# willow-ahrens/ChainPartitioners.jl

Measured on AMD Instinct MI355X. Metric: partitions/sec, DynamicTotalSplitter(AffineConnectivityModel{Int64}(0,0,0,1)), K=64, higher is better.
Workload: dtype int64; 1 GPU; config 3: DynamicTotalSplitter(AffineConnectivityModel{Int64}(0,0,0,1)) on suitesparse_shaped CSR (seeded SplitMix64 generator, tests/synth.py), n=10000000 rows, nnz=100000000, K=64; one independent partition per GPU; n=10000000, nnz=100000000, K=64, includes_oracle_build=True, device_block_pool=True

## Files before the change

chainpartitioners.jl_amd/csrc/capi.hip:

```cpp
#include "csr.hpp"
#include "model.hpp"
#include "dp.hpp"
#include "weight.hpp"
#include "sym.hpp"
#include <cmath>
#include <memory>

using namespace cpk;

namespace cpk {

__global__ void __launch_bounds__(256) k_range_counts(int64_t nq, const int64_t *__restrict__ P, const int64_t *__restrict__ Rr,
                                                      const int64_t *__restrict__ pos, const int32_t *__restrict__ prev,
                                                      const int64_t *__restrict__ fpos, const int32_t *__restrict__ flast,
                                                      unsigned long long *__restrict__ nets, unsigned long long *__restrict__ selfnets)
{
    int64_t i = blockIdx.x;
    if (i >= nq) return;
    __shared__ int64_t sh[256];
    int64_t p = P[i], r = Rr[i];
    int64_t stride = (int64_t)gridDim.y * 256, start = (int64_t)blockIdx.y * 256 + threadIdx.x;
    int64_t c = 0;
    if (r > p) {
        int64_t q0 = pos[p], q1 = pos[r];
// ... 54 lines not shown
        hp[i] = j[i] - 1; hr[i] = jp[i] - 1;
    }
    DBuf<int64_t> dP((size_t)nq), dR((size_t)nq), dK, dN, dS;
    DBuf<TC> dO((size_t)nq);
    CP_HIP(hipMemcpyAsync(dP.p, hp.data(), sizeof(int64_t) * (size_t)nq, hipMemcpyHostToDevice, s));
    CP_HIP(hipMemcpyAsync(dR.p, hr.data(), sizeof(int64_t) * (size_t)nq, hipMemcpyHostToDevice, s));
    if (k) { dK.alloc((size_t)nq); CP_HIP(hipMemcpyAsync(dK.p, k, sizeof(int64_t) * (size_t)nq, hipMemcpyHostToDevice, s)); }
    if (has_nets) {
        dN.alloc((size_t)nq);
        CP_HIP(hipMemsetAsync(dN.p, 0, dN.bytes(), s));
        if (need_self) { dS.alloc((size_t)nq); CP_HIP(hipMemsetAsync(dS.p, 0, dS.bytes(), s)); }
        int64_t per = nq > 0 ? A->N / nq : 0;
        unsigned gy = (unsigned)(per / 65536 + 1);
        if (gy > 2048) gy = 2048;
        ProfScope ps(PROF_QUERY, s, 0.0);
        hipLaunchKernelGGL(k_range_counts, dim3((unsigned)nq, gy), dim3(256), 0, s, nq, dP.p, dR.p, A->pos.p, A->prev.p,
                           need_self ? A->fpos.p : nullptr, need_self ? A->flast.p : nullptr, (unsigned long long *)dN.p,
                           need_self ? (unsigned long long *)dS.p : nullptr);
    }
    HostModel<TC> HM;
    build_dev_model<TC>(mdl, HM, s);
    hipLaunchKernelGGL(HIP_KERNEL_NAME(k_apply_model<TC>), dim3((unsigned)cdiv(nq, 256)), dim3(256), 0, s, nq, dP.p, dR.p,
                       k ? dK.p : nullptr, A->pos.p, has_nets ? dN.p : nullptr, need_self ? dS.p : nullptr, HM.d, dO.p);
    CP_HIP(hipGetLastError());
    CP_HIP(hipMemcpyAsync(out, dO.p, sizeof(TC) * (size_t)nq, hipMemcpyDeviceToHost, s));
    CP_HIP(hipStreamSynchronize(s));
    prof_collect();
    return CP_OK;
}

static int64_t fld(int64_t a, int64_t b)
{
    int64_t q = a / b, r = a % b;
    if (r != 0 && ((r < 0) != (b < 0))) q -= 1;
    return q;
}
static double fld(double a, int64_t b) { return std::floor(a / (double)b); }
static int64_t max_identity(int64_t) { return INT64_MIN; }
static double max_identity(double) { return -INFINITY; }
static void also_f64(const int64_t *lo, const int64_t *hi, double *lo_f64, double *hi_f64) { *lo_f64 = (double)*lo; *hi_f64 = (double)*hi; }
static void also_f64(const double *, const double *, double *, double *) {}

template <typename TC>
static int32_t oracle_eval_into(cp_csr_t A, const cp_model_t *model, const cp_rowpart_t *Pi, int64_t nq, const int64_t *j, const int64_t *jp,
                                const int64_t *k, TC *out)
{
    const bool i64 = std::is_same<TC, int64_t>::value;
    return cp_oracle_eval(A, model, Pi, CP_HINT_STEP, nq, j, jp, k, i64 ? (int64_t *)out : nullptr, i64 ? nullptr : (double *)out);
}

static const struct { const char *name; int64_t *var; bool kept; } g_stats[] = {
    {"spec_redo", &g_spec_redo, false}, {"poison_hits", &g_poison_hits, false}, {"fix_trips", &g_fix_trips, false},
    {"fix_edges", &g_fix_edges, false}, {"fix_items", &g_fix_items, false}, {"bn_sym_layers", &g_bn_sym_layers, true},
    {"own_split_tiles", &g_own_split_tiles, false},
};
static void stats_reset(bool all) { for (const auto &c : g_stats) if (all || !c.kept) *c.var = 0; }

enum OptRule { OPT_PLAIN, OPT_BOOL, OPT_CLAMP, OPT_POW2 };
constexpr int64_t NOLIM_LO = INT64_MIN, NOLIM_HI = INT64_MAX;
static const struct Opt { const char *name; int64_t *var; OptRule rule; int64_t lo, hi; } g_options[] = {
    {"force_brute", &g_opt_force_brute, OPT_PLAIN, 0, 0}, {"brute_max_n", &g_opt_brute_max_n, OPT_PLAIN, 0, 0}, {"dbg", &g_opt_dbg, OPT_PLAIN, 0, 0},
    {"short_t", &g_opt_short_t, OPT_PLAIN, 0, 0}, {"short_e", &g_opt_short_e, OPT_PLAIN, 0, 0}, {"ra_cache", &g_opt_ra_cache, OPT_PLAIN, 0, 0},
    {"leaf", &g_opt_leaf, OPT_PLAIN, 0, 0}, {"block_tables", &g_opt_block_tables, OPT_PLAIN, 0, 0}, {"nospec", &g_opt_nospec, OPT_PLAIN, 0, 0},
    {"rpass_small_tau", &g_opt_rpass_small_tau, OPT_PLAIN, 0, 0}, {"fixed_point", &g_opt_fixed_point, OPT_PLAIN, 0, 0},
    {"bn_wave", &g_opt_bn_wave, OPT_PLAIN, 0, 0},
    {"poison", &g_opt_poison, OPT_PLAIN, 0, 0},
    {"pool", &g_opt_pool, OPT_BOOL, 0, 0},
    {"own_blk", &g_opt_own_blk, OPT_BOOL, 0, 0},
    {"own_split", &g_opt_own_split, OPT_BOOL, 0, 0},
    {"lws", &g_opt_lws, OPT_BOOL, 0, 0},
    {"gap_tau", &g_opt_gap_tau, OPT_CLAMP, NOLIM_LO, 20}, {"gap_min", &g_opt_gap_min, OPT_CLAMP, 8, NOLIM_HI}, {"gap_nr", &g_opt_gap_nr, OPT_CLAMP, 1, 2},
    {"force_max", &g_opt_force_max, OPT_CLAMP, 0, NOLIM_HI}, {"rpass_cap", &g_opt_rpass_cap, OPT_CLAMP, 1, NOLIM_HI},
    {"own_min", &g_opt_own_min, OPT_CLAMP, 64, NOLIM_HI}, {"bn_chunk", &g_opt_bn_chunk, OPT_CLAMP, 1, NOLIM_HI},
    {"bn_slack", &g_opt_bn_slack, OPT_CLAMP, 0, NOLIM_HI}, {"bn_run", &g_opt_bn_run, OPT_CLAMP, 2, NOLIM_HI},
    {"rpass_ch", &g_opt_rpass_ch, OPT_POW2, 16, 4096}, {"setup_bs", &g_opt_setup_bs, OPT_POW2, 64, 1024}, {"lws_leaf", &g_opt_lws_leaf, OPT_POW2, 256, 2048},
};
static int64_t opt_value(const Opt &o, int64_t value)
{
    switch (o.rule) {
    case OPT_BOOL: return value ? 1 : 0;
    case OPT_CLAMP: return value < o.lo ? o.lo : value > o.hi ? o.hi : value;
    case OPT_POW2: { int64_t v = o.lo; while (v < value && v < o.hi) v <<= 1; return v; }
    default: return value;
    }
}

}

extern "C" {

const char *cp_last_error(void) { return g_last_error.c_str(); }
int32_t cp_version(void) { return 100; }

int32_t cp_device_count(void)
{
    int c = 0;
    if (hipGetDeviceCount(&c) != hipSuccess) return 0;
    return c;
}

static int32_t csr_create_impl(int64_t m, int64_t n, int64_t N, const int64_t *colptr, const int64_t *rowval,
                               int32_t device, bool on_device, cp_csr_t *out)
{
    return guarded([&]() -> int32_t {
        CP_REQUIRE(out && colptr && (rowval || N == 0), CP_EINVAL, "null argument");
        CP_REQUIRE(m >= 0 && n >= 0 && N >= 0, CP_EINVAL, "negative dimension");
        CP_REQUIRE(n < (int64_t)1 << 30 && m < (int64_t)1 << 30 && N < ((int64_t)1 << 31) - 65536, CP_EINVAL,
                   "dimensions exceed the 32-bit link-array layout");
        CP_REQUIRE(cp_device_count() > 0, CP_EHIP, "no HIP device visible: libchainpart has no CPU fallback");
        CP_HIP(hipSetDevice(device));
        std::unique_ptr<cp_csr_s> A(new cp_csr_s());
        A->device = device; A->m = m; A->n = n; A->N = N;
        CP_HIP(hipStreamCreate(&A->stream));
        A->own_stream = true;
        csr_upload(A.get(), colptr, rowval, on_device);
        *out = A.release();
        return CP_OK;
    });
}

int32_t cp_csr_create(int64_t m, int64_t n, int64_t N, const int64_t *colptr, const int64_t *rowval, int32_t device, cp_csr_t *out)
{
// ... 510 lines not shown
```

chainpartitioners.jl_amd/csrc/dp.hpp:

```cpp
#pragma once
#include "csr.hpp"
#include "model.hpp"

struct cp_dp_s {
    cp_csr_s *A = nullptr;
    int64_t K = 0;
    int32_t combine = 0, order = 0;
    bool fast = false, fast_bn = false, need_self = false;
    void *work = nullptr;
    cpk::DBuf<int32_t> ptr;
    int64_t rlo = 0, rhi = 0;
    int64_t wwin = 0;
    std::vector<int64_t> lay_lo, lay_hi;
    virtual ~cp_dp_s() = default;
    virtual int32_t step_layer(int64_t k, const void *cst_prev_device, void *cst_cur_device) = 0;
    virtual int32_t block_tables(int32_t *nplanes_out, int64_t *opt_out, int64_t *nets_out, int64_t *selfnets_out) = 0;
};

namespace cpk {

using DpBase = ::cp_dp_s;

struct DpWindow {
    int64_t w = 0;
// ... 37 lines not shown
                         int64_t wwin = 0, int64_t p_lo0 = 0, int64_t p_hi0 = -1, const int32_t *j0 = nullptr,
                         const BnPattern *pat = nullptr);
extern int64_t g_opt_bn_wave, g_opt_bn_run, g_opt_bn_slack;
extern int64_t g_opt_bn_chunk;

template <typename TC>
int32_t run_dyn_constrained(cp_csr_s *A, int64_t K, int32_t g, int32_t order, const cp_model_t *mdl, const cp_rowpart_t *Pi,
                            const cp_model_t *w, int64_t wi, double wf, int64_t *spl_out);
template <typename TC>
int32_t run_seq_eval(cp_csr_s *A, const cp_model_t *mdl, const cp_rowpart_t *Pi, int64_t nq, const int64_t *j, const int64_t *jp,
                     const int64_t *k, TC *out);

template <typename TC>
int32_t run_plaid_eval(cp_csr_s *A, const cp_model_t *mdl, const cp_rowpart_t *Pi, int64_t nq, const int64_t *j, const int64_t *jp,
                       const int64_t *k, TC *out);
template <typename TC>
int32_t run_plaid_dynamic(cp_csr_s *A, int64_t K, int32_t combine, int32_t order, const cp_model_t *mdl, const cp_rowpart_t *Pi,
                          int64_t *spl_out);

template <typename TC>
bool pack_dynamic_scan(hipStream_t s, int64_t n, int64_t wmax, const TC *Ftab, TC *cst1, int64_t *spl1);

extern int64_t g_opt_lws, g_opt_lws_leaf;
bool lws_ok(const cp_csr_s *A, const cp_model_t *mdl, const cp_model_t *w, int64_t wi, double wf);
template <typename TC>
int32_t run_pack_lws(cp_csr_s *A, const DevModel<TC> &M, const WaveletDev &wnet, const WaveletDev &wself, const cp_model_t *w, int64_t wi,
                     double wf, TC *cst1, int64_t *spl1);

extern int64_t g_opt_gap_nr;
extern int64_t g_opt_gap_tau, g_opt_gap_min;
extern int64_t g_opt_poison, g_poison_hits;
void dp_round_scans_test(const int32_t *a, int64_t na, int64_t na_max, const int32_t *b, int64_t nb, int64_t nb_max, int two, int64_t capT, int64_t capNT,
                         int err_in, int reps, int64_t *offs_out, int64_t *toffs_out, int64_t *res);
void dp_fix_merge_test(const cp_model_t *model, int64_t ntask, const int64_t *toffs, const int64_t *part_v, const int32_t *part_p, const int32_t *part_nn,
                       const int32_t *part_nl, const int32_t *tile_s, const int32_t *tile_s2, const int32_t *anchor, const int32_t *anchor2, const int32_t *row,
                       const int32_t *plane, int64_t n, int reps, int32_t *p_out, int32_t *nn_out, int32_t *nl_out, int64_t *res);
extern int64_t g_fix_trips, g_fix_edges;
extern int64_t g_fix_items;
extern int64_t g_opt_leaf;
extern int64_t g_opt_block_tables;
extern int64_t g_opt_ra_cache;
extern int64_t g_opt_fixed_point;
extern int64_t g_opt_nospec;
extern int64_t g_spec_redo;
extern int64_t g_opt_rpass_small_tau;
extern int64_t g_opt_force_max;
extern int64_t g_opt_setup_bs;
extern int64_t g_opt_rpass_cap;
extern int64_t g_opt_rpass_ch;
extern int64_t g_opt_own_min;
extern int64_t g_opt_own_blk;
extern int64_t g_opt_own_split;
extern int64_t g_own_split_tiles;
void dp_own_split_test(cp_csr_s *A, int32_t *vpos_out, int32_t *vsa_out, int32_t *vnext_out, int64_t *res);
extern int64_t g_opt_short_t, g_opt_short_e;
extern int64_t g_opt_force_brute;
extern int64_t g_opt_brute_max_n;
extern int64_t g_opt_dbg;
enum DbgBit : int64_t {
    DBG_PRINT_ROUNDS = 8,
    DBG_NO_INTERIOR = 32,
    DBG_NO_OWN_TILES = 64,
    DBG_POISON = 128,
    DBG_POISON_ZERO = 256,
    DBG_GAP_ALL_SPECIAL = 512,
    DBG_MISPREDICT = 1024,
    DBG_TINY_BUFFERS = 2048,
    DBG_COUNT_NONTRIVIAL = 4096,
    DBG_COMBINE_BY_SLOT = 16384,
    DBG_RA_ROWMAJOR = 262144,
    DBG_NO_FORCE_OWN = 524288,
    DBG_WIN_NO_RA_CACHE = 1048576,
    DBG_WIN_NO_MIR_CACHE = 2097152,
    DBG_BN_NO_HINT2 = 4194304,
    DBG_MIR_ROWMAJOR = 8388608,
    DBG_RA_ALL_LEVELS = 33554432,
    DBG_BN_NO_HINT_STARTS = 33554432,
};

}
```

chainpartitioners.jl_amd/csrc/dp_brute.hip:

```cpp
#include "csr.hpp"
#include "model.hpp"
#include "dp.hpp"

namespace cpk {

int64_t g_opt_force_brute = 0;
int64_t g_opt_short_t = 8, g_opt_short_e = 64;
int64_t g_opt_own_min = 64;
int64_t g_opt_own_blk = 1;
int64_t g_opt_own_split = 1;
int64_t g_own_split_tiles = 0;
int64_t g_opt_rpass_ch = 256;
int64_t g_opt_rpass_small_tau = 4;
int64_t g_opt_force_max = 1024;
int64_t g_opt_setup_bs = 1024;
int64_t g_opt_rpass_cap = 200;
int64_t g_opt_nospec = 0, g_spec_redo = 0;
int64_t g_opt_gap_tau = 6, g_opt_gap_min = 64, g_opt_gap_nr = 2;
int64_t g_opt_ra_cache = 1;
int64_t g_opt_leaf = 1, g_opt_block_tables = 0;
int64_t g_opt_poison = 0, g_poison_hits = 0;
int64_t g_fix_trips = 0, g_fix_edges = 0, g_fix_items = 0;
int64_t g_opt_fixed_point = 0;
int64_t g_opt_brute_max_n = 200000;
int64_t g_opt_dbg = 0;

template <typename TC>
__global__ void __launch_bounds__(256) k_brute_layer(int64_t n, int64_t r_lo, int64_t r_hi, const int64_t *__restrict__ pos,
                                                     const int32_t *__restrict__ next, const int64_t *__restrict__ fpos,
                                                     const int32_t *__restrict__ flast, DevModel<TC> M, TC alpha,
                                                     int32_t g, const TC *__restrict__ W, TC *__restrict__ cst,
                                                     int32_t *__restrict__ ptr)
{
    int64_t wave = ((int64_t)blockIdx.x * blockDim.x + threadIdx.x) >> 6;
    int lane = threadIdx.x & 63;
    int64_t r0 = r_lo + wave * 64;
    if (r0 > r_hi) return;
    int64_t r = r0 + lane;
    bool live = r <= r_hi;
    int64_t rtop = r0 + 63 < r_hi ? r0 + 63 : r_hi;
    int64_t nn = 0, nl = 0;
    TC best = (TC)0;
    int64_t bp = -1;
    bool self = (M.kind == CP_MODEL_HYPEREDGE_CUT);
    int32_t rr = (int32_t)r;
    for (int64_t p = rtop; p >= 0; p--) {
        if (p < n) {
            bool step = live && (r > p);
            int64_t q0 = pos[p], q1 = pos[p + 1];
            for (int64_t q = q0; q < q1; q++) {
                int32_t nx = next[q];
                if (step) nn += (nx >= rr);
            }
            if (self) {
                int64_t s0 = fpos[p], s1 = fpos[p + 1];
                for (int64_t sidx = s0; sidx < s1; sidx++) {
                    int32_t la = flast[sidx];
                    if (step) nl += (la < rr);
                }
            }
        }
        if (live && r >= p) {
            TC f = dm_apply(M, alpha, r - p, pos[r] - pos[p], nn, nl);
            TC v = comb(g, W[p], f);
// ... 25 lines not shown
```

chainpartitioners.jl_amd/csrc/dp_total.hip:

```cpp
#include "csr.hpp"
#include "model.hpp"
#include "dp.hpp"
#include <algorithm>

namespace cpk {

template <typename TC>
__device__ __forceinline__ TC dm_apply_affine(const DevModel<TC> &m, TC alpha, int64_t nv, int64_t np, int64_t nn, int64_t nl)
{
    TC v = cadd(cadd(alpha, cmulc(nv, m.p[CP_P_VERTEX])), cmulc(np, m.p[CP_P_PIN]));
    if (m.kind == CP_MODEL_CONNECTIVITY) return cadd(v, cmulc(nn, m.p[CP_P_NET]));
    if (m.kind == CP_MODEL_HYPEREDGE_CUT) return cadd(cadd(v, cmulc(nl, m.p[CP_P_SELF_NET])), cmulc(nn - nl, m.p[CP_P_CUT_NET]));
    return v;
}
#define dm_apply dm_apply_affine

constexpr int LT = 256;
constexpr int NBMAX = 31;
constexpr int SPLIT_BMIN = 8;
constexpr int SPLIT_NB = NBMAX - SPLIT_BMIN;

__device__ __forceinline__ int64_t prow(int64_t r, int64_t n)
{
    int t = __ffsll((long long)r) - 1;
// ... 771 lines not shown
        if (hi > re) hi = re;
        if (hi > n + 1) hi = n + 1;
        gap_hi[tile] = (int32_t)hi;
    }
    }
}

__global__ void __launch_bounds__(256) k_blk_order(const RoundCounts *__restrict__ rc, const int4 *__restrict__ rec, const int32_t *__restrict__ brank,
                                                   const int64_t *__restrict__ bstart, int32_t *__restrict__ border, int4 *__restrict__ srec,
                                                   int32_t *__restrict__ bcnt)
{
    const int64_t ntile = rc->NT;
    for (int64_t tile = (int64_t)blockIdx.x * blockDim.x + threadIdx.x; tile < ntile; tile += (int64_t)gridDim.x * blockDim.x) {
        const int4 r = rec[tile];
        const int32_t c = r.x / LT, rk = brank[tile];
        const int64_t slot = bstart[c] + rk;
        border[slot] = (int32_t)tile;
        srec[slot] = r;
        if (rk == 0) bcnt[c] = 0;
    }
}

template <typename TC, bool HYP, bool GAP>
__global__ void __launch_bounds__(256) k_lpass_own(int isA, const RoundCounts *__restrict__ rc, const int32_t *__restrict__ border,
                                                   const int32_t *__restrict__ a_pos, const int32_t *__restrict__ a_next,
                                                   const int32_t *__restrict__ a_fpos, const int32_t *__restrict__ a_flast,
                                                   int32_t *__restrict__ a_tileS, int32_t *__restrict__ a_tileS2, const int4 *__restrict__ a_rec,
                                                   const int4 *__restrict__ a_srec, const TC *__restrict__ W, DevModel<TC> M, TC alpha, Best<TC, HYP> *__restrict__ part,
                                                   int tau, const int32_t *__restrict__ gap_hi, uint8_t *__restrict__ spec, int force_spec,
                                                   Best<TC, HYP> *__restrict__ sub, int32_t *__restrict__ spv,
                                                   const int32_t *__restrict__ a_col, const int32_t *__restrict__ a_ffirst,
                                                   const int32_t *__restrict__ a_vnext, const int32_t *__restrict__ a_vpos,
                                                   const int32_t *__restrict__ a_vsa, int64_t vstride)
{
    int lane = threadIdx.x & 63;
    int64_t tile = (int64_t)blockIdx.x * 4 + __builtin_amdgcn_readfirstlane(threadIdx.x >> 6);
    if (tile >= rc->NT) return;
    const int4 vrec = border ? a_srec[tile] : a_rec[tile];
    if (border) tile = border[tile];
    const int32_t rw = __builtin_amdgcn_readfirstlane(vrec.w);
    const int4 rec = make_int4(__builtin_amdgcn_readfirstlane(vrec.x), __builtin_amdgcn_readfirstlane(vrec.y), __builtin_amdgcn_readfirstlane(vrec.z), rw);
    int head = rw & 1;
    int32_t tl = (rw >> 2) & 255;
    int32_t acc[4], acc2[4] = {0, 0, 0, 0}, sk[4], sk2[4];
    __shared__ int32_t s_es_all[4][2][SMAX + 1], s_v_all[4][2][SMAX + 1];
    __shared__ int32_t s_cnt_all[4];
    int32_t(*s_es)[SMAX + 1] = s_es_all[threadIdx.x >> 6], (*s_v)[SMAX + 1] = s_v_all[threadIdx.x >> 6];
    int ns = 0;
    if (GAP && (rw & 2)) {
        int32_t *s_cnt = &s_cnt_all[threadIdx.x >> 6];
        if (lane == 0) *s_cnt = 0;
        __threadfence_block();
        int32_t rL = rec.y - (1 << tau), hi1 = gap_hi[tile] - 1;
        interior_stream<true, true>(a_next, a_pos, rec.x, tl, hi1, lane, acc, sk, head, rL, hi1, s_es[0], s_v[0], s_cnt, 0);
        if (HYP) interior_stream<false, true>(a_flast, a_fpos, rec.x, tl, rL + 1, lane, acc2, sk2, head, rL, hi1, s_es[0], s_v[0], s_cnt, 1);
        __threadfence_block();
        ns = *s_cnt;
        if (force_spec) ns = SMAX + 1;
        if (ns > 0 && ns <= SMAX) {
            if (lane < ns) {
                const int32_t q = s_es[0][lane];
                const bool k1 = s_v[0][lane] < 0;
                s_es[0][lane] = rec.x - (k1 ? a_ffirst[q] : a_col[q]);
            }
            __threadfence_block();
        }
    } else if (!HYP && !GAP) {
        const int sb = rw >> 10;
        const int64_t so = sb ? (int64_t)(sb - SPLIT_BMIN) * vstride : 0;
        interior_stream<true>(sb ? a_vnext : a_next, sb ? a_vpos + so : a_pos, rec.x, tl, rec.y, lane, acc, sk, head, 0, 0, nullptr, nullptr, nullptr, 0,
                              sb ? a_vsa + so : (const int32_t *)nullptr);
#pragma unroll
        for (int k = 0; k < 4; k++) { const int32_t e = lane + 64 * k; sk[k] = (a_pos + (rec.x - tl))[(uint32_t)(tl - (e < tl ? e : tl)) & 255u]; }
    } else {
        interior_stream<true>(a_next, a_pos, rec.x, tl, rec.y, lane, acc, sk, head);
        if (HYP) interior_stream<false>(a_flast, a_fpos, rec.x, tl, rec.y, lane, acc2, sk2, head);
    }
    TC wv[4];
#pragma unroll
    for (int k = 0; k < 4; k++) { const int32_t e = lane + 64 * k; wv[k] = (W + (rec.x - tl))[(uint32_t)(tl - (e < tl ? e : tl)) & 255u]; }
    int sel = tl >> 6;
    if (lane == (tl & 63)) {
        a_tileS[tile] = sel == 0 ? acc[0] : sel == 1 ? acc[1] : sel == 2 ? acc[2] : acc[3];
        if (HYP) a_tileS2[tile] = sel == 0 ? acc2[0] : sel == 1 ? acc2[1] : sel == 2 ? acc2[2] : acc2[3];
    }
    Best<TC, HYP> cand[4];
#pragma unroll
    for (int k = 0; k < 4; k++) {
        int32_t e = lane + 64 * k;
        best_clear(cand[k]);
        if (e <= tl && !(head && isA && e == 0)) {
            int32_t p = rec.x - e;
            TC fv = dm_apply(M, alpha, (int64_t)(rec.y - p), (int64_t)(rec.z - sk[k]), (int64_t)acc[k], (int64_t)acc2[k]);
            cand[k].v = cadd(wv[k], fv); cand[k].p = p; cand[k].nn = acc[k]; best_set_nl(cand[k], acc2[k]);
        }
    }
    if (GAP && ns > SMAX) {
        if (lane == 0) spec[tile] = 255;
        return;
    }
    if (!GAP || ns == 0) {
        Best<TC, HYP> best; best_clear(best);
#pragma unroll
        for (int k = 0; k < 4; k++) best = better(best, cand[k]);
        for (int o = 32; o > 0; o >>= 1) {
            int src = (lane + o) & 63;
            Best<TC, HYP> c; best_clear(c); c.v = shfl64(best.v, src); c.p = __shfl(best.p, src); c.nn = __shfl(best.nn, src);
            if (HYP) best_set_nl(c, __shfl(best_nl(best), src));
            bool take = (best.p < 0) ? (c.p >= 0) : (c.p >= 0 && (c.v < best.v || (c.v == best.v && c.p > best.p)));
            if (lane + o < 64 && take) best = c;
        }
        if (lane == 0) { part[tile] = best; if (GAP) spec[tile] = 0; }
        return;
    }
    __threadfence_block();
    if (lane < ns) {
        int32_t es_i = s_es[0][lane]; int rank = 0;
        for (int j = 0; j < ns; j++) { int32_t es_j = s_es[0][j]; rank += (es_j < es_i) || (es_j == es_i && j < lane); }
// ... 2038 lines not shown
            dim3 sgrid((unsigned)cdiv(R.ntask, sbs));
            if (!R.isA) {
                int64_t mx = 1;
                for (int bb = R.tau + 1; bb < nbits; bb++) mx = std::max<int64_t>(mx, R.tbase[bb + 1] - R.tbase[bb]);
                sgrid = dim3((unsigned)cdiv(mx, sbs), (unsigned)std::max(1, nbits - R.tau - 1));
            }
            hipLaunchKernelGGL(HIP_KERNEL_NAME(k_setup_short<TC, HYP>), sgrid, dim3(sbs), 0, s, R, Wk.opt.p, Wk.nnopt.p, Wk.nlopt.p, Wk.cr.p, Wk.crl.p, A->pos32.p,
                               A->next.p, if_hyp<HYP>(A->fpos32.p), if_hyp<HYP>(A->flast.p), W, M, alpha, Wk.tdesc.p, Wk.tb.p, Wk.len.p, Wk.tS0l.p, &rc->nlong,
                               (int32_t)g_opt_short_t, (int32_t)g_opt_short_e, own_tiles ? Wk.o_tdesc.p : (int4 *)nullptr, Wk.o_tb.p, Wk.o_rlen.p, Wk.o_ntl.p,
                               Wk.o_tS0l.p, &rc->nown, &rc->own_steps, (int32_t)(forced ? 2 : gap ? g_opt_gap_min : g_opt_own_min),
                               (int32_t)std::min<size_t>(Wk.o_ntl.n, (size_t)INT32_MAX), &rc->err, Wk.fin.p, Wk.last_s0.p,
                               (g_opt_dbg & DBG_COUNT_NONTRIVIAL) ? &rc->_pad : (int32_t *)nullptr, Wk.w_anch.p, Wk.w_anch2.p, pzp, oblk);
        }
        RoundCounts P;
        if (spec) {
            P = Wk.pred[(size_t)rd];
            if (Wk.pred_scale != 1.0) {
                auto sc = [&](int64_t v) { return (int64_t)((double)v * Wk.pred_scale) + (v > 0 ? 1 : 0); };
                P.nlong = (int32_t)sc(P.nlong); P.nown = (int32_t)sc(P.nown); P.T = sc(P.T); P.NT = sc(P.NT);
                P.own_steps = (unsigned long long)sc((int64_t)P.own_steps);
            }
            if ((g_opt_dbg & DBG_MISPREDICT) && (rd & 1)) { P.nown = 0; P.NT = 0; P.nlong = 0; P.T = 0; }
            Wk.ensure_own((size_t)grow(P.NT));
            Wk.ensure_flat((size_t)grow(P.T));
        }
        {
            ProfScope ps(PROF_SCAN, s, 12.0 * (double)R.ntask);
            const bool tiny = spec && (g_opt_dbg & DBG_TINY_BUFFERS);
            const int64_t capT = spec ? (tiny ? (int64_t)64 : (int64_t)Wk.loc.n) : INT64_MAX, capNT = spec ? (tiny ? (int64_t)1 : (int64_t)Wk.o_rec.n) : INT64_MAX;
            const int64_t nm = std::min<int64_t>(R.ntask, (int64_t)Wk.o_ntl.n);
            if (R.ntask <= LB_MAX) {
                launch_round_scans(rc, Wk.len.p, Wk.offs.p, R.ntask, Wk.o_ntl.p, Wk.o_toffs.p, nm, own_tiles, capT, capNT, Wk.scanws, s);
            } else {
                exclusive_scan_i32_devn(Wk.len.p, Wk.offs.p, &rc->nlong, R.ntask, &rc->T, Wk.scratch, s);
                if (own_tiles) exclusive_scan_i32_devn(Wk.o_ntl.p, Wk.o_toffs.p, &rc->nown, nm, &rc->NT, Wk.scratch, s);
                hipLaunchKernelGGL(k_round_finish, dim3(1), dim3(1), 0, s, rc, capT, capNT);
            }
        }
        if (!spec) {
            CP_HIP(hipMemcpyAsync(&P, rc, sizeof(P), hipMemcpyDeviceToHost, s));
            CP_HIP(hipStreamSynchronize(s));
            Wk.ensure_own((size_t)P.NT);
            Wk.ensure_flat((size_t)P.T);
        }
        used[(size_t)rd] = P;
        if (g_opt_dbg & DBG_PRINT_ROUNDS) fprintf(stderr, "round isA=%d tau=%d ntask=%lld %s long=%d own=%d T=%lld NT=%lld nontrivial=%d\n", R.isA, R.tau, (long long)R.ntask,
                                   spec ? "predicted" : "exact", P.nlong, P.nown, (long long)P.T, (long long)P.NT, P._pad);
        if (P.nown > 0 && P.NT > 0) {
            const int64_t gNT = spec ? (int64_t)Wk.o_rec.n : P.NT, gown = spec ? grow(P.nown) : P.nown;
            poison_fill(s, {{Wk.o_part.p, Wk.o_part.bytes()}, {Wk.o_tileS.p, Wk.o_tileS.bytes()}, {Wk.o_rec.p, Wk.o_rec.bytes()}, {Wk.o_srec.p, Wk.o_srec.bytes()},
                            {if_hyp<HYP>(Wk.o_tileS2.p), Wk.o_tileS2.bytes()}, {Wk.o_items.p, Wk.o_items.bytes()}, {Wk.o_item_of.p, Wk.o_item_of.bytes()},
                            {Wk.o_trec.p, Wk.o_trec.bytes()}});
            const unsigned mgrid = (unsigned)std::min<int64_t>(cdiv(gNT, 256), 8192);
            const int split = !(split_layer && !gap && !R.isA) ? 0 : R.tau + 1 >= SPLIT_BMIN ? 1 : 2;
            split_mode[(size_t)rd] = (int8_t)split;
            if (split && !Wk.split.built) {
                ProfScope ps(PROF_LINKS, s, 8.0 * (double)A->N + 16.0 * (double)(nbits - SPLIT_BMIN) * (double)(n + 1));
                split_build(A, Wk.split, Wk.scratch);
            }
            hipLaunchKernelGGL(k_own_map, dim3(mgrid), dim3(256), 0, s, rc, Wk.o_toffs.p, Wk.o_tdesc.p, Wk.o_rlen.p, Wk.o_rec.p, Wk.o_task.p,
                               Wk.o_tb.p, gap ? Wk.o_hi.p : (int32_t *)nullptr, R.tau, n, oblk, oblk ? Wk.b_cnt.p : (int32_t *)nullptr, Wk.o_brank.p,
                               gap ? (int2 *)nullptr : Wk.o_items.p, Wk.o_item_of.p, split);
            {
                ProfScope ps(gap ? PROF_GAPSTREAM : PROF_OWN, s, own_bytes(R.tau, split != 0, (double)P.own_steps));
                if (oblk) {
                    exclusive_scan_i32_lb(Wk.b_cnt.p, Wk.b_start.p, Wk.b_n.p, Wk.b_nblk, nullptr, Wk.scanws, s);
                    hipLaunchKernelGGL(k_blk_order, dim3(mgrid), dim3(256), 0, s, rc, Wk.o_rec.p, Wk.o_brank.p, Wk.b_start.p, Wk.o_border.p, Wk.o_srec.p, Wk.b_cnt.p);
                }
                hipLaunchKernelGGL(HIP_KERNEL_NAME(gap ? k_lpass_own<TC, HYP, true> : k_lpass_own<TC, HYP, false>), dim3((unsigned)cdiv(gNT, 4)), dim3(256), 0, s,
                                   R.isA, rc,
                                   oblk ? Wk.o_border.p : (const int32_t *)nullptr, A->pos32.p, A->next.p, if_hyp<HYP>(A->fpos32.p), if_hyp<HYP>(A->flast.p),
                                   Wk.o_tileS.p, Wk.o_tileS2.p, Wk.o_rec.p, Wk.o_srec.p, W, M, alpha, recs<HYP>(Wk.o_part), R.tau, Wk.o_hi.p, Wk.o_spec.p,
                                   (int)((g_opt_dbg & DBG_GAP_ALL_SPECIAL) != 0), recs<HYP>(Wk.o_sub), Wk.o_spv.p, A->col.p, if_hyp<HYP>(A->ffirst.p),
                                   split ? Wk.split.vnext.p : (const int32_t *)nullptr, Wk.split.vpos.p, Wk.split.vsa.p, (int64_t)(n + 1));
            }
            note(rd, 0, gap ? PROF_GAPSTREAM : PROF_OWN, R.tau, split != 0);
            if (gap) {
                {
                    ProfScope ps(PROF_CARRY, s, 12.0 * (double)P.NT);
                    const int32_t *ntp = reinterpret_cast<const int32_t *>(&rc->NT);
                    exclusive_scan_i32_lb(Wk.o_tileS.p, Wk.o_tilePS.p, ntp, (int64_t)Wk.o_tileS.n, nullptr, Wk.scanws, s);
                    if (hyp) exclusive_scan_i32_lb(Wk.o_tileS2.p, Wk.o_tilePS2.p, ntp, (int64_t)Wk.o_tileS.n, nullptr, Wk.scanws, s);
                }
                ProfScope ps(PROF_GAP, s, 24.0 * (double)P.NT);
                const int nchunk = (int)std::max<int64_t>(1, ((int64_t)2 << R.tau) / 64);
                const size_t ncap = Wk.o_rec.n / GAPSEG + 2;
                Wk.g_list.ensure(ncap); Wk.g_slot.ensure(2 * ncap);
                Wk.g_seg.ensure((2 * ncap) * (size_t)nchunk * 64 * sizeof(GapSegRec<TC, true>));
                Wk.g_slow.ensure((size_t)gown * (size_t)nchunk + 64); Wk.g_sslow.ensure((2 * ncap) * (size_t)nchunk + 64);
                CP_REQUIRE((int64_t)gown * nchunk < INT32_MAX && (int64_t)(2 * ncap) * nchunk < INT32_MAX, CP_EINTERNAL, "gap work index beyond 32 bits");
                const int gnr = (g_opt_gap_nr >= 2 && nchunk >= 2) ? 2 : 1;
                unsigned gg = (unsigned)std::min<int64_t>(cdiv(gown * cdiv((int64_t)nchunk, gnr), 4), 16384);
                unsigned gs_grid = (unsigned)std::min<int64_t>(cdiv((int64_t)(2 * ncap) * nchunk, 4), 8192);
                unsigned gm = (unsigned)std::min<int64_t>(cdiv((int64_t)ncap * nchunk, 4), 4096);
                const unsigned gslow_grid = 2048;
                launch_gap<TC, HYP>(s, A, Wk, R.tau, nchunk, gnr, rc, n, W, M, alpha, gg, gs_grid, gm, gslow_grid, oblk);
            } else {
                ProfScope ps(PROF_FIX, s, 24.0 * (double)P.NT);
                launch_fix_own<TC, HYP>(s, rc, Wk.o_toffs.p, recs<HYP>(Wk.o_part), Wk.o_tdesc.p, Wk.o_tb.p, if_hyp<HYP>(Wk.o_tS0l.p), Wk.o_tileS.p,
                                        if_hyp<HYP>(Wk.o_tileS2.p), M, Wk.opt.p, Wk.nnopt.p, if_hyp<HYP>(Wk.nlopt.p), n, Wk.o_items.p, Wk.o_item_of.p, Wk.o_trec.p,
                                        Wk.o_tick.p, spec ? grow(P.NT) : P.NT, gown);
            }
            CP_HIP(hipGetLastError());
        }
        if (P.nlong <= 0 || P.T <= 0) continue;
        const int64_t gtile = spec ? (int64_t)Wk.tileS.n : cdiv(P.T, LT);
        poison_fill(s, {{Wk.loc.p, Wk.loc.bytes()}, {if_hyp<HYP>(Wk.loc2.p), Wk.loc2.bytes()}, {Wk.partL.p, Wk.partL.bytes()}, {Wk.partR.p, Wk.partR.bytes()},
                        {Wk.tileS.p, Wk.tileS.bytes()}, {if_hyp<HYP>(Wk.tileS2.p), Wk.tileS2.bytes()}});
// ... 37 lines not shown
            CP_REQUIRE(need <= 25, CP_EINTERNAL, "leaf pass: more outer planes than counters");
            const int32_t lcap = (gaps && g_opt_gap_tau >= LEAF_T) ? (int32_t)std::max<int64_t>(g_opt_gap_min, 2) : INT32_MAX;
            LeafArgs<TC, HYP> L{};
            L.n = n; L.g0 = g0; L.ngroups = g1 - g0 + 1; L.c0 = c0; L.c1 = c1; L.nbits = nbits; L.planes = (int32_t)(g_opt_block_tables != 0);
            L.pos = A->pos32.p; L.prev = A->prev.p; L.next = A->next.p; L.col = A->col.p;
            L.fpos = if_hyp<HYP>(A->fpos32.p); L.flast = if_hyp<HYP>(A->flast.p); L.ffirst = if_hyp<HYP>(A->ffirst.p);
            L.lpos = if_hyp<HYP>(A->lpos32.p); L.lfirst = if_hyp<HYP>(A->lfirst.p);
            L.opt = Wk.opt.p; L.nnopt = Wk.nnopt.p; L.nlopt = if_hyp<HYP>(Wk.nlopt.p); L.fin = Wk.fin.p; L.fin_stamp = Wk.fin_stamp;
            L.W = W; L.M = M; L.alpha = alpha; L.cst = cst_out; L.ptr = ptr_out; L.G = G;
            L.anchM = Wk.leaf_anch.p; L.anchM2 = if_hyp<HYP>(Wk.leaf_anch2.p); L.lcap = lcap; L.err = &Wk.rc.p->err; L.pz = pzp;
            constexpr int WPB = LeafWPB<HYP>::v;
            hipLaunchKernelGGL(HIP_KERNEL_NAME(need <= 18 ? k_leaf<TC, HYP, 18> : k_leaf<TC, HYP, 25>), dim3((unsigned)cdiv(L.ngroups, WPB)), dim3(64 * WPB), 0, s, L);
            CP_HIP(hipGetLastError());
        }
    }
    {
        ProfScope ps(PROF_COMBINE, s, 24.0 * (double)(leaf ? (n >> LEAF_T) + 1 : n + 1));
        const int64_t c0 = rlo > 0 ? rlo : 0, c1 = rhi < n ? rhi : n;
        const int64_t r0 = leaf ? (c0 + LEAF_G - 1) >> LEAF_T : c0, r1 = leaf ? c1 >> LEAF_T : c1;
        const int lvl = (!leaf && (g_opt_dbg & DBG_COMBINE_BY_SLOT)) ? (2 * (c1 - c0 + 1) >= n + 1) : 0;
        const int sh = leaf ? LEAF_T : 0;
        const int32_t *nl = if_hyp<HYP>(Wk.nlopt.p);
        if (c1 >= c0 && r1 >= r0) {
            const unsigned cgrid = (unsigned)cdiv(lvl ? n + 1 : r1 - r0 + 1, 256);
            if (G.win) hipLaunchKernelGGL(HIP_KERNEL_NAME(k_combine_win<TC>), dim3(cgrid), dim3(256), 0, s, lvl, G, n, r0, r1, A->pos32.p, Wk.opt.p, Wk.nnopt.p, nl, W, M,
                                          alpha, cst_out, ptr_out, sh, pzp);
            else hipLaunchKernelGGL(HIP_KERNEL_NAME(k_combine<TC>), dim3(cgrid), dim3(256), 0, s, lvl, n, r0, r1, nbits, A->pos32.p, Wk.opt.p, Wk.nnopt.p, nl, W, M, alpha,
                                    cst_out, ptr_out, sh, pzp);
        }
    }
    CP_HIP(hipGetLastError());
    std::vector<RoundCounts> got((size_t)NR);
    int32_t pz_hits[2] = {0, 0};
    CP_HIP(hipMemcpyAsync(got.data(), Wk.rc.p, sizeof(RoundCounts) * (size_t)NR, hipMemcpyDeviceToHost, s));
    if (pzp) CP_HIP(hipMemcpyAsync(pz_hits, pzp, sizeof(pz_hits), hipMemcpyDeviceToHost, s));
    CP_HIP(hipStreamSynchronize(s));
    bool ok = true;
    for (int rd = 0; rd < NR; rd++) {
        const RoundCounts &g = got[(size_t)rd], &u = used[(size_t)rd];
        CP_REQUIRE(!(g.err && !spec && !any_forced), CP_EINTERNAL, "DP work list overflow");
        if (g.err) ok = false;
        if (g.nown > 0 && g.NT > 0 && !(u.nown > 0 && u.NT > 0)) ok = false;
        if (g.nlong > 0 && g.T > 0 && !(u.nlong > 0 && u.T > 0)) ok = false;
    }
    if (pzp) {
        g_poison_hits += pz_hits[0];
        CP_REQUIRE(!(ok && pz_hits[0] > 0), CP_EINTERNAL, "a DP layer that is not redone read plane cells nobody wrote (poison mode)");
    }
    if (ok) Wk.b_dirty = false;
    Wk.t_dirty = false;
    if (ok) for (int rd = 0; rd < NR; rd++) { g_fix_trips += got[(size_t)rd].n_trips; g_fix_edges |= got[(size_t)rd].n_edge; }
    if (ok) for (int rd = 0; rd < NR; rd++) {
        const RoundCounts &g = got[(size_t)rd];
        if (g.nown > 0 && g.NT > 0) g_own_split_tiles += split_mode[(size_t)rd] == 1 ? g.NT : split_mode[(size_t)rd] == 2 ? g.n_split : 0;
    }
    for (int rd = 0; rd < NR; rd++) g_fix_items += got[(size_t)rd].n_items;
    if (ok) {
        for (auto &pt : patches) {
            const RoundCounts &g = got[(size_t)pt.rd];
            if (pt.idx < g_prof_pending.size())
                g_prof_pending[pt.idx].bytes = pt.kind == 0 ? own_bytes(pt.tau, pt.split, (double)g.own_steps) : (double)g.T * step_bytes;
        }
        Wk.pred = got; Wk.pred_ok = true; Wk.pred_rlo = rlo; Wk.pred_rhi = rhi; Wk.pred_win = G.win; Wk.pred_w = G.w;
        if (allow_force && 2 * (rhi - rlo + 1) >= Wk.force_rows) {
            Wk.force_own.resize((size_t)NR, 0);
            Wk.force_rows = rhi - rlo + 1;
            for (int rd = 1; rd < NR; rd++) {
                const RoundCounts &g = got[(size_t)rd];
                if (g.nlong > 0) Wk.force_own[(size_t)rd] = g.nlong <= g_opt_force_max;
            }
        }
    }
    return ok;
}

template <typename TC>
void dp_total_layer(cp_csr_s *A, const DevModel<TC> &M, TC alpha, const TC *W, TC *cst_out, int32_t *ptr_out, void *work_,
                    int64_t rlo, int64_t rhi, int64_t wwin)
{
    auto &Wk = *reinterpret_cast<LayerWork<TC> *>(work_);
    int64_t n = A->n;
    bool hyp = M.kind == CP_MODEL_HYPEREDGE_CUT;
    int nbits = 1;
    while (((int64_t)1 << nbits) <= n) nbits++;
    CP_REQUIRE(nbits <= NBMAX, CP_EINVAL, "n exceeds the bit-plane budget");
    if (Wk.n != n || Wk.hyp != hyp) {
        Wk.n = -1; Wk.nbits = nbits; Wk.hyp = hyp;
        Wk.forget();
        Wk.o_rec.release(); Wk.loc.release();
        size_t plane = (size_t)nbits * (size_t)(n + 1);
        Wk.opt.alloc(plane); Wk.nnopt.alloc(plane); Wk.cr.alloc(plane);
        if (hyp) { Wk.nlopt.alloc(plane); Wk.crl.alloc(plane); }
        CP_HIP(hipMemsetAsync(Wk.opt.p, 0, Wk.opt.bytes(), A->stream));
        CP_HIP(hipMemsetAsync(Wk.nnopt.p, 0, Wk.nnopt.bytes(), A->stream));
        CP_HIP(hipMemsetAsync(Wk.cr.p, 0, Wk.cr.bytes(), A->stream));
        if (hyp) { CP_HIP(hipMemsetAsync(Wk.nlopt.p, 0, Wk.nlopt.bytes(), A->stream)); CP_HIP(hipMemsetAsync(Wk.crl.p, 0, Wk.crl.bytes(), A->stream)); }
        int64_t mx = n;
        for (int tau = 0; tau < nbits; tau++) { RoundDesc R; make_round(R, false, tau, nbits, n, 0, n); if (R.ntask > mx) mx = R.ntask; }
        for (int tau = 0; tau < nbits; tau++) mx = std::max<int64_t>(mx, ((n >> (tau + 1)) + 1) * (int64_t)(nbits - 1 - tau));
        mx = std::max<int64_t>(mx, 2 * n + nbits);
        Wk.max_tasks = mx > 0 ? mx : 1;
        size_t mt = (size_t)Wk.max_tasks;
        Wk.tdesc.alloc(mt); Wk.len.alloc(mt); Wk.tb.alloc(mt); Wk.offs.alloc(mt + 1);
        if (hyp) Wk.tS0l.alloc(mt);
        int64_t mmin = std::max<int64_t>(2, std::min(g_opt_own_min, g_opt_gap_tau >= 0 ? g_opt_gap_min : g_opt_own_min));
        size_t mo = (size_t)(2 * n / mmin + 64) * (size_t)nbits + 1024;
        if (mo > mt) mo = mt;
// ... 79 lines not shown
```

Measured before the change: 2.596 partitions/s.

## Extend split-link streaming to gap-stream tiles in the total-cost DP

Enables the split link structure (vnext/vpos/vsa per bit level) for gap-mode own tiles in non-hypergraph layers, so long tiles stream through shortened link chains instead of the full next/pos arrays. It also replaces the per-lane column lookups that turn special entries into offsets with a ballot/popcount rank over the in-register keys, and reloads sk from pos afterwards. A new gap_split option (on by default) and a separate split-tile counter are added. This may require building the split structure in layers that previously skipped it, and adds a serial per-entry ballot loop.

```diff
diff --git a/chainpartitioners.jl_amd/csrc/capi.hip b/chainpartitioners.jl_amd/csrc/capi.hip
--- a/chainpartitioners.jl_amd/csrc/capi.hip
+++ b/chainpartitioners.jl_amd/csrc/capi.hip
@@ -130,7 +130,7 @@
 static const struct { const char *name; int64_t *var; bool kept; } g_stats[] = {
     {"spec_redo", &g_spec_redo, false}, {"poison_hits", &g_poison_hits, false}, {"fix_trips", &g_fix_trips, false},
     {"fix_edges", &g_fix_edges, false}, {"fix_items", &g_fix_items, false}, {"bn_sym_layers", &g_bn_sym_layers, true},
-    {"own_split_tiles", &g_own_split_tiles, false},
+    {"own_split_tiles", &g_own_split_tiles, false}, {"gap_split_tiles", &g_gap_split_tiles, false},
 };
 static void stats_reset(bool all) { for (const auto &c : g_stats) if (all || !c.kept) *c.var = 0; }
 
@@ -146,6 +146,7 @@
     {"pool", &g_opt_pool, OPT_BOOL, 0, 0},
     {"own_blk", &g_opt_own_blk, OPT_BOOL, 0, 0},
     {"own_split", &g_opt_own_split, OPT_BOOL, 0, 0},
+    {"gap_split", &g_opt_gap_split, OPT_BOOL, 0, 0},
     {"lws", &g_opt_lws, OPT_BOOL, 0, 0},
     {"gap_tau", &g_opt_gap_tau, OPT_CLAMP, NOLIM_LO, 20}, {"gap_min", &g_opt_gap_min, OPT_CLAMP, 8, NOLIM_HI}, {"gap_nr", &g_opt_gap_nr, OPT_CLAMP, 1, 2},
     {"force_max", &g_opt_force_max, OPT_CLAMP, 0, NOLIM_HI}, {"rpass_cap", &g_opt_rpass_cap, OPT_CLAMP, 1, NOLIM_HI},
diff --git a/chainpartitioners.jl_amd/csrc/dp.hpp b/chainpartitioners.jl_amd/csrc/dp.hpp
--- a/chainpartitioners.jl_amd/csrc/dp.hpp
+++ b/chainpartitioners.jl_amd/csrc/dp.hpp
@@ -113,6 +113,8 @@
 extern int64_t g_opt_own_blk;
 extern int64_t g_opt_own_split;
 extern int64_t g_own_split_tiles;
+extern int64_t g_opt_gap_split;
+extern int64_t g_gap_split_tiles;
 void dp_own_split_test(cp_csr_s *A, int32_t *vpos_out, int32_t *vsa_out, int32_t *vnext_out, int64_t *res);
 extern int64_t g_opt_short_t, g_opt_short_e;
 extern int64_t g_opt_force_brute;
diff --git a/chainpartitioners.jl_amd/csrc/dp_brute.hip b/chainpartitioners.jl_amd/csrc/dp_brute.hip
--- a/chainpartitioners.jl_amd/csrc/dp_brute.hip
+++ b/chainpartitioners.jl_amd/csrc/dp_brute.hip
@@ -10,6 +10,8 @@
 int64_t g_opt_own_blk = 1;
 int64_t g_opt_own_split = 1;
 int64_t g_own_split_tiles = 0;
+int64_t g_opt_gap_split = 1;
+int64_t g_gap_split_tiles = 0;
 int64_t g_opt_rpass_ch = 256;
 int64_t g_opt_rpass_small_tau = 4;
 int64_t g_opt_force_max = 1024;
diff --git a/chainpartitioners.jl_amd/csrc/dp_total.hip b/chainpartitioners.jl_amd/csrc/dp_total.hip
--- a/chainpartitioners.jl_amd/csrc/dp_total.hip
+++ b/chainpartitioners.jl_amd/csrc/dp_total.hip
@@ -847,18 +847,38 @@
         if (lane == 0) *s_cnt = 0;
         __threadfence_block();
         int32_t rL = rec.y - (1 << tau), hi1 = gap_hi[tile] - 1;
-        interior_stream<true, true>(a_next, a_pos, rec.x, tl, hi1, lane, acc, sk, head, rL, hi1, s_es[0], s_v[0], s_cnt, 0);
+        const int sb = HYP ? 0 : rw >> 10;
+        const int64_t so = sb ? (int64_t)(sb - SPLIT_BMIN) * vstride : 0;
+        interior_stream<true, true>(sb ? a_vnext : a_next, sb ? a_vpos + so : a_pos, rec.x, tl, hi1, lane, acc, sk, head, rL, hi1, s_es[0], s_v[0], s_cnt, 0,
+                                    sb ? a_vsa + so : (const int32_t *)nullptr);
         if (HYP) interior_stream<false, true>(a_flast, a_fpos, rec.x, tl, rL + 1, lane, acc2, sk2, head, rL, hi1, s_es[0], s_v[0], s_cnt, 1);
         __threadfence_block();
         ns = *s_cnt;
         if (force_spec) ns = SMAX + 1;
         if (ns > 0 && ns <= SMAX) {
-            if (lane < ns) {
-                const int32_t q = s_es[0][lane];
-                const bool k1 = s_v[0][lane] < 0;
-                s_es[0][lane] = rec.x - (k1 ? a_ffirst[q] : a_col[q]);
+            if (HYP) {
+                if (lane < ns) {
+                    const int32_t q = s_es[0][lane];
+                    const bool k1 = s_v[0][lane] < 0;
+                    s_es[0][lane] = rec.x - (k1 ? a_ffirst[q] : a_col[q]);
+                }
+            } else {
+                int32_t es = 0;
+                for (int i = 0; i < ns; i++) {
+                    const int32_t q = s_es[0][i];
+                    int32_t c = 0;
+#pragma unroll
+                    for (int k = 0; k < 4; k++) c += (int32_t)__popcll(__ballot(lane + 64 * k <= tl && sk[k] > q));
+                    if (lane == i) es = c;
+                }
+                __threadfence_block();
+                if (lane < ns) s_es[0][lane] = es;
             }
             __threadfence_block();
+        }
+        if (!HYP) {
+#pragma unroll
+            for (int k = 0; k < 4; k++) { const int32_t e = lane + 64 * k; sk[k] = (a_pos + (rec.x - tl))[(uint32_t)(tl - (e < tl ? e : tl)) & 255u]; }
         }
     } else if (!HYP && !GAP) {
         const int sb = rw >> 10;
@@ -3003,8 +3023,8 @@
                             {if_hyp<HYP>(Wk.o_tileS2.p), Wk.o_tileS2.bytes()}, {Wk.o_items.p, Wk.o_items.bytes()}, {Wk.o_item_of.p, Wk.o_item_of.bytes()},
                             {Wk.o_trec.p, Wk.o_trec.bytes()}});
             const unsigned mgrid = (unsigned)std::min<int64_t>(cdiv(gNT, 256), 8192);
-            const int split = !(split_layer && !gap && !R.isA) ? 0 : R.tau + 1 >= SPLIT_BMIN ? 1 : 2;
-            split_mode[(size_t)rd] = (int8_t)split;
+            const int split = !(split_layer && !R.isA && (!gap || g_opt_gap_split)) ? 0 : R.tau + 1 >= SPLIT_BMIN ? 1 : 2;
+            split_mode[(size_t)rd] = (int8_t)(gap ? -split : split);
             if (split && !Wk.split.built) {
                 ProfScope ps(PROF_LINKS, s, 8.0 * (double)A->N + 16.0 * (double)(nbits - SPLIT_BMIN) * (double)(n + 1));
                 split_build(A, Wk.split, Wk.scratch);
@@ -3148,7 +3168,10 @@
     if (ok) for (int rd = 0; rd < NR; rd++) { g_fix_trips += got[(size_t)rd].n_trips; g_fix_edges |= got[(size_t)rd].n_edge; }
     if (ok) for (int rd = 0; rd < NR; rd++) {
         const RoundCounts &g = got[(size_t)rd];
-        if (g.nown > 0 && g.NT > 0) g_own_split_tiles += split_mode[(size_t)rd] == 1 ? g.NT : split_mode[(size_t)rd] == 2 ? g.n_split : 0;
+        if (g.nown > 0 && g.NT > 0) {
+            const int sm = split_mode[(size_t)rd];
+            (sm < 0 ? g_gap_split_tiles : g_own_split_tiles) += std::abs(sm) == 1 ? g.NT : std::abs(sm) == 2 ? g.n_split : 0;
+        }
     }
     for (int rd = 0; rd < NR; rd++) g_fix_items += got[(size_t)rd].n_items;
     if (ok) {
```

Result: faster. 2.665 partitions/s, median of 6 (+2.6%).
